# BurntSushi/aho-corasick

Hardware: NVIDIA H100
Metric: haystack_scan_throughput (higher is better)
Workload: dtype u8

## Files before the change

aho-corasick_b200/csrc/acb_api.cu:

```cuda
#include <cuda_runtime.h>

#include <algorithm>
#include <chrono>
#include <cstdio>
#include <cstdlib>
#include <cstring>
#include <atomic>
#include <pthread.h>
#include <condition_variable>
#include <functional>
#include <mutex>
#include <thread>
#include <new>
#include <vector>

#include "../../include/acb200.h"
#include "../../include/acb200_debug.h"
#include "acb_build.hpp"
#include "acb_comm.hpp"
#include "acb_device.cuh"

using acb::DfaDev;
using acb::HostDfa;

namespace {

#define CK(expr)                                                                       \
  do {                                                                                 \
    cudaError_t e_ = (expr);                                                           \
    if (e_ != cudaSuccess) {                                                           \
      std::fprintf(stderr, "acb200: CUDA error %s at %s:%d: %s\n", cudaGetErrorName(e_), \
                   __FILE__, __LINE__, cudaGetErrorString(e_));                        \
      return ACG_E_CUDA;                                                               \
    }                                                                                  \
  } while (0)

struct Workspace {
  cudaStream_t stream = nullptr, copy_stream = nullptr;
  cudaEvent_t ev0 = nullptr, ev1 = nullptr, ev2 = nullptr, ev3 = nullptr;
  uint64_t cap = 0;
  uint64_t* d_keys[2] = {nullptr, nullptr};
  uint32_t* d_pids[2] = {nullptr, nullptr};
  unsigned long long* d_counter = nullptr;
  unsigned long long* h_counter = nullptr;
  void* d_temp = nullptr;
  size_t temp_bytes = 0;
  uint64_t* h_keys = nullptr;
  uint32_t* h_pids = nullptr;
  uint64_t h_cap = 0;
  uint8_t* d_hay = nullptr;
  uint64_t d_hay_cap = 0;
  uint64_t* d_scratch = nullptr;
  uint8_t* d_flags = nullptr;
  void* d_temp2 = nullptr;
  size_t temp2_bytes = 0;
  uint64_t chain_cap = 0;
  uint64_t* d_seq = nullptr;
  uint64_t seq_cap = 0;
  uint64_t* h_seq = nullptr;
  uint64_t h_seq_cap = 0;
  acg_stats stats{};
  uint8_t* h_stage[2] = {nullptr, nullptr};
  uint64_t h_stage_cap = 0;
  cudaEvent_t stage_ev[2] = {nullptr, nullptr};
};

}

// ... 29 lines not shown
  int device = -1;
  uint32_t* d_trans = nullptr;
  uint8_t* d_classes = nullptr;
  uint32_t* d_moff = nullptr;
  uint32_t* d_mpids = nullptr;
  uint32_t* d_plens = nullptr;
  uint16_t* d_depth16 = nullptr;
  DfaDev dev{};
  int engine_override = ACG_ENGINE_AUTO;
  uint64_t pipeline_chunk = 64ull << 20;
  mutable bool bytescan_inert = false;
  uint32_t experiment = 0;
  mutable std::mutex mu;
  static constexpr size_t kMaxWorkspaces = 4;
  mutable std::vector<Workspace*> ws_all, ws_free;
  mutable std::condition_variable ws_cv;
  mutable acg_stats last_stats{};
};

namespace {

thread_local Workspace* tls_ws = nullptr;
thread_local const acg_dfa* tls_stats_owner = nullptr;
thread_local acg_stats tls_stats{};
Workspace& cur_ws() { return *tls_ws; }

int init_workspace(Workspace& w) {
  CK(cudaStreamCreateWithFlags(&w.stream, cudaStreamNonBlocking));
  CK(cudaStreamCreateWithFlags(&w.copy_stream, cudaStreamNonBlocking));
  CK(cudaEventCreate(&w.ev0));
  CK(cudaEventCreate(&w.ev1));
  CK(cudaEventCreate(&w.ev2));
  CK(cudaEventCreate(&w.ev3));
  CK(cudaMalloc(&w.d_counter, 64));
  CK(cudaMallocHost(&w.h_counter, 64));
  return ACG_OK;
}

void destroy_workspace(Workspace& w) {
  if (w.stream) cudaStreamSynchronize(w.stream);
  for (int i = 0; i < 2; ++i) { cudaFree(w.d_keys[i]); cudaFree(w.d_pids[i]); }
  cudaFree(w.d_counter); cudaFree(w.d_temp); cudaFree(w.d_hay); cudaFree(w.d_seq);
  cudaFree(w.d_scratch); cudaFree(w.d_flags); cudaFree(w.d_temp2);
  if (w.h_counter) cudaFreeHost(w.h_counter);
  if (w.h_keys) cudaFreeHost(w.h_keys);
  if (w.h_pids) cudaFreeHost(w.h_pids);
  if (w.h_seq) cudaFreeHost(w.h_seq);
  for (int i = 0; i < 2; ++i) {
    if (w.h_stage[i]) cudaFreeHost(w.h_stage[i]);
    if (w.stage_ev[i]) cudaEventDestroy(w.stage_ev[i]);
  }
  if (w.ev0) cudaEventDestroy(w.ev0);
  if (w.ev1) cudaEventDestroy(w.ev1);
  if (w.ev2) cudaEventDestroy(w.ev2);
  if (w.ev3) cudaEventDestroy(w.ev3);
  if (w.stream) cudaStreamDestroy(w.stream);
  if (w.copy_stream) cudaStreamDestroy(w.copy_stream);
}

struct WsLease {
  const acg_dfa* a;
  Workspace* w = nullptr;
  Workspace* prev;
  int rc = ACG_OK;
  explicit WsLease(const acg_dfa* a_) : a(a_), prev(tls_ws) {
    std::unique_lock<std::mutex> lk(a->mu);
    for (;;) {
      if (!a->ws_free.empty()) { w = a->ws_free.back(); a->ws_free.pop_back(); break; }
// ... 581 lines not shown
    CK(cudaEventRecord(w.ev0, w.stream));
    CK(acb::launch_walk_overlapping(a->dev, p, w.stream));
    CK(cudaEventRecord(w.ev1, w.stream));
    CK(cudaMemcpyAsync(w.h_counter, w.d_counter, 8, cudaMemcpyDeviceToHost, w.stream));
    CK(cudaStreamSynchronize(w.stream));
    cur_ws().stats.launches += 1;
    const uint64_t want = *w.h_counter;
    if (want > w.cap) { cap = want + want / 8 + 1024; continue; }
    res->n = want;
    cur_ws().stats.raw_matches = want;
    float ms = 0;
    cudaEventElapsedTime(&ms, w.ev0, w.ev1);
    cur_ws().stats.scan_ms = ms;
    if (want > 1) {
      size_t tb = w.temp_bytes;
      const int end_bit = std::min(64, acb::kTieBits + bits_for(n_bytes + 1));
      CK(cudaEventRecord(w.ev2, w.stream));
      CK(acb::sort_pairs(w.d_temp, tb, w.d_keys[0], w.d_keys[1], w.d_pids[0], w.d_pids[1], want, end_bit,
                         w.stream));
      CK(cudaEventRecord(w.ev3, w.stream));
      CK(cudaStreamSynchronize(w.stream));
      cudaEventElapsedTime(&ms, w.ev2, w.ev3);
      cur_ws().stats.order_ms = ms;
      cur_ws().stats.launches += 8;
      res->sorted_buf = 1;
    } else {
      res->sorted_buf = 0;
    }
    return ACG_OK;
  }
  return ACG_E_NOMEM;
}

int enqueue_prefilter_range(const acg_dfa* a, const uint8_t* d_hay, uint64_t readable,
                            uint64_t span_start, uint64_t span_end, uint64_t scan_lo,
                            uint64_t scan_hi, int mode, int dev_sms) {
  Workspace& w = cur_ws();
  const PrefilterPlan& pf = a->pf;
  const uintptr_t base = reinterpret_cast<uintptr_t>(d_hay);
  uint64_t lo = scan_lo + ((16 - ((base + scan_lo) & 15)) & 15);
  const uint64_t limit = std::min<uint64_t>(scan_hi, readable >= 20 ? readable - 20 : 0);
  uint64_t hi = lo;
  if (limit > lo) hi = lo + ((limit - lo) & ~15ull);
  if (lo > scan_hi) { lo = scan_hi; hi = scan_hi; }
  acb::PrefilterLaunch p;
  p.hay = d_hay;
  p.hay_len = readable;
  p.span_start = span_start;
  p.span_end = span_end;
  p.bitmap = a->d_bitmap;
  p.log_bits = pf.log_bits;
  p.k = pf.k;
  p.stride = pf.stride;
  p.geom = pf.wide ? 1 : 0;
  p.pair = 0;
  p.dyn = (a->experiment & ACG_EXP_STATIC_TILES) ? 0 : ((a->experiment & ACG_EXP_GLOBAL_TILES) ? 2 : 1);
  p.kmask = pf.kmask;
  p.fold = pf.fold;
  p.mult = pf.mult;
  p.mult3 = pf.mult3;
  p.key_shift = pf.key_shift;
  p.shift = pf.shift;
  p.dense = pf.dense ? 1 : 0;
  p.brute = pf.brute ? 1 : 0;
  p.mode = mode == 1 ? 1 : 0;
  p.first_only = mode == 2 ? 1 : 0;
  p.dup_shift = pf.dup_shift;
  p.scan_lo = scan_lo;
  p.scan_hi = scan_hi;
  p.region_lo = lo;
  p.region_hi = hi;
  p.keys = w.d_keys[0];
  p.pids = w.d_pids[0];
  p.counter = w.d_counter;
  p.cap = w.cap;
  p.bs_n = 0;
  for (int i = 0; i < 3; ++i) { p.bs_needle[i] = 0; p.bs_back[i] = 0; }
  if (pf.bs_n && !a->bytescan_inert && !(a->experiment & ACG_EXP_NO_BYTESCAN)) {
    p.bs_n = pf.bs_n;
    for (uint32_t i = 0; i < pf.bs_n; ++i) { p.bs_needle[i] = uint32_t(pf.bs_byte[i]) * 0x01010101u; p.bs_back[i] = pf.bs_back[i]; }
    CK(acb::launch_bytescan(a->dev, p, dev_sms, w.stream));
  } else {
    if (p.dyn == 2) CK(cudaMemsetAsync(w.d_counter + 2, 0, 8, w.stream));
    CK(acb::launch_prefilter(a->dev, p, dev_sms, w.stream));
  }
  cur_ws().stats.launches += 1;
  return ACG_OK;
}

int order_tuples(const acg_dfa* a, uint64_t want, uint64_t n_bytes, TupleResult* res) {
  Workspace& w = cur_ws();
  res->n = want;
  cur_ws().stats.raw_matches = want;
  if (want > 1) {
    size_t tb = w.temp_bytes;
    const int end_bit = std::min(64, acb::kTieBits + bits_for(n_bytes + 1));
    float ms = 0;
    CK(cudaEventRecord(w.ev2, w.stream));
    CK(acb::sort_pairs(w.d_temp, tb, w.d_keys[0], w.d_keys[1], w.d_pids[0], w.d_pids[1], want, end_bit,
                       w.stream));
    CK(cudaEventRecord(w.ev3, w.stream));
    CK(cudaStreamSynchronize(w.stream));
    cudaEventElapsedTime(&ms, w.ev2, w.ev3);
    cur_ws().stats.order_ms = ms;
    cur_ws().stats.launches += 8;
    res->sorted_buf = 1;
  } else {
    res->sorted_buf = 0;
  }
  return ACG_OK;
}

class CopyPool {
 public:
  static CopyPool& get() {
    static std::once_flag once;
    std::call_once(once, [] { pthread_atfork(nullptr, nullptr, [] { instance().store(nullptr); }); });
    CopyPool* p = instance().load(std::memory_order_acquire);
    if (!p) {
      CopyPool* fresh = new CopyPool;
      if (instance().compare_exchange_strong(p, fresh)) p = fresh;
    }
    return *p;
  }
  void copy(uint8_t* dst, const uint8_t* src, size_t n) {
    if (n < (4u << 20) || workers_.empty()) { std::memcpy(dst, src, n); return; }
    std::unique_lock<std::mutex> lk(mu_);
    busy_cv_.wait(lk, [&] { return !active_; });
    active_ = true;
    dst_ = dst; src_ = src; n_ = n;
    next_.store(0);
    pending_ = int(workers_.size());
    ++epoch_;
    cv_.notify_all();
    done_cv_.wait(lk, [&] { return pending_ == 0; });
    active_ = false;
    busy_cv_.notify_one();
  }

 private:
  static std::atomic<CopyPool*>& instance() {
    static std::atomic<CopyPool*> p{nullptr};
// ... 34 lines not shown
  std::atomic<size_t> next_{0};
  int pending_ = 0;
  uint64_t epoch_ = 0;
  bool active_ = false;
};

bool is_pageable_host(const void* p) {
  cudaPointerAttributes attr;
  if (cudaPointerGetAttributes(&attr, p) != cudaSuccess) { cudaGetLastError(); return false; }
  return attr.type == cudaMemoryTypeUnregistered;
}

int ensure_stage(Workspace& w, uint64_t bytes) {
  if (bytes <= w.h_stage_cap) return ACG_OK;
  for (int i = 0; i < 2; ++i) {
    if (w.h_stage[i]) { cudaFreeHost(w.h_stage[i]); w.h_stage[i] = nullptr; }
    CK(cudaMallocHost(&w.h_stage[i], bytes));
    if (!w.stage_ev[i]) CK(cudaEventCreateWithFlags(&w.stage_ev[i], cudaEventDisableTiming));
  }
  w.h_stage_cap = bytes;
  return ACG_OK;
}

int run_prefilter(const acg_dfa* a, const uint8_t* d_hay, uint64_t readable, uint64_t span_start,
                  uint64_t span_end, int mode, TupleResult* res, const uint8_t* h_hay = nullptr,
                  uint64_t scan_lo = UINT64_MAX, uint64_t scan_hi = UINT64_MAX) {
  if (scan_lo == UINT64_MAX) { scan_lo = span_start; scan_hi = span_end; }
  Workspace& w = cur_ws();
  const uint64_t n_bytes = span_end - span_start;
  if (n_bytes >= (1ull << (64 - acb::kTieBits))) return ACG_E_INVALID_ARG;
  int dev_sms = 132;
  cudaDeviceGetAttribute(&dev_sms, cudaDevAttrMultiProcessorCount, a->device);
  uint64_t cap = std::max<uint64_t>(w.cap, std::max<uint64_t>(1 << 20, (scan_hi - scan_lo) / 256));
  bool copied = h_hay == nullptr;
  for (int attempt = 0; attempt < 8; ++attempt) {
    int rc = ensure_tuple_cap(w, cap);
    if (rc) return rc;
    CK(cudaMemsetAsync(w.d_counter, 0, 16, w.stream));
    CK(cudaEventRecord(w.ev0, w.stream));
    if (copied) {
      if ((rc = enqueue_prefilter_range(a, d_hay, readable, span_start, span_end, scan_lo, scan_hi, mode,
                                        dev_sms)))
        return rc;
    } else {
      const uint64_t chunk = a->pipeline_chunk;
      const uint64_t tail = std::min<uint64_t>(a->h.max_pattern_len, 1u << 30) + 64;
      uint64_t scanned = span_start;
      const bool staged = span_end - span_start >= std::min<uint64_t>(8u << 20, chunk) && is_pageable_host(h_hay + span_start);
      if (staged && (rc = ensure_stage(w, std::min<uint64_t>(chunk, span_end - span_start)))) return rc;
      bool stage_used[2] = {false, false};
      int stage_i = 0;
      CK(cudaEventRecord(w.ev2, w.copy_stream));
      for (uint64_t c0 = span_start; c0 < span_end; c0 += chunk) {
        const uint64_t c1 = std::min(span_end, c0 + chunk);
        const uint8_t* src = h_hay + c0;
        if (staged) {
          if (stage_used[stage_i]) CK(cudaEventSynchronize(w.stage_ev[stage_i]));
          CopyPool::get().copy(w.h_stage[stage_i], h_hay + c0, size_t(c1 - c0));
          src = w.h_stage[stage_i];
        }
        CK(cudaMemcpyAsync(const_cast<uint8_t*>(d_hay) + c0, src, c1 - c0, cudaMemcpyHostToDevice,
                           w.copy_stream));
        if (staged) {
          CK(cudaEventRecord(w.stage_ev[stage_i], w.copy_stream));
          stage_used[stage_i] = true;
          stage_i ^= 1;
        }
        CK(cudaEventRecord(w.ev3, w.copy_stream));
        CK(cudaStreamWaitEvent(w.stream, w.ev3, 0));
        const uint64_t upto = c1 == span_end ? span_end : (c1 > scanned + tail ? c1 - tail : scanned);
        if (upto > scanned || c1 == span_end) {
          if ((rc = enqueue_prefilter_range(a, d_hay, c1 == span_end ? readable : c1, span_start, span_end,
                                            scanned, upto, mode, dev_sms)))
            return rc;
          scanned = upto;
        }
      }
      copied = true;
    }
    CK(cudaEventRecord(w.ev1, w.stream));
    CK(cudaMemcpyAsync(w.h_counter, w.d_counter, 16, cudaMemcpyDeviceToHost, w.stream));
    CK(cudaStreamSynchronize(w.stream));
    const uint64_t want = w.h_counter[0];
    cur_ws().stats.candidates = w.h_counter[1];
    if (a->pf.bs_n && !a->bytescan_inert && scan_hi - scan_lo >= (1u << 16) && w.h_counter[1] > (scan_hi - scan_lo) / 64)
      a->bytescan_inert = true;
    float ms = 0;
    cudaEventElapsedTime(&ms, w.ev0, w.ev1);
    cur_ws().stats.scan_ms = ms;
    if (want > w.cap) { cap = want + want / 8 + 1024; continue; }
    return order_tuples(a, want, n_bytes, res);
  }
  return ACG_E_NOMEM;
}

int ensure_chain(Workspace& w, uint64_t n) {
  if (n <= w.chain_cap) return ACG_OK;
  if (w.d_scratch) cudaFree(w.d_scratch);
  if (w.d_flags) cudaFree(w.d_flags);
  if (w.d_temp2) cudaFree(w.d_temp2);
  w.d_scratch = nullptr; w.d_flags = nullptr; w.d_temp2 = nullptr; w.chain_cap = 0;
  const uint64_t cap = std::max<uint64_t>(n, 1 << 16);
  CK(cudaMalloc(&w.d_scratch, cap * 8));
  CK(cudaMalloc(&w.d_flags, cap));
  size_t t1 = 0, t2 = 0;
  CK(acb::scan_max_u64(nullptr, t1, w.d_scratch, cap, w.stream));
  CK(acb::select_flagged(nullptr, t2, w.d_keys[0], w.d_pids[0], w.d_flags, w.d_keys[1], w.d_pids[1],
                         w.d_counter, cap, w.stream));
  w.temp2_bytes = std::max(t1, t2);
  CK(cudaMalloc(&w.d_temp2, std::max<size_t>(w.temp2_bytes, 16)));
  w.chain_cap = cap;
  return ACG_OK;
}

int run_chain(const acg_dfa* a, int mode, TupleResult* r) {
  Workspace& w = cur_ws();
  if (r->n == 0) return ACG_OK;
  int rc = ensure_chain(w, r->n);
  if (rc) return rc;
  const int src = r->sorted_buf, dst = 1 - src;
  acb::ChainLaunch c;
  c.keys = w.d_keys[src];
  c.pids = w.d_pids[src];
  c.pattern_lens = a->d_plens;
// ... 1107 lines not shown
```

aho-corasick_b200/csrc/acb_device.cuh:

```cuda
#pragma once
#include <cuda_runtime.h>
#include <stdint.h>

namespace acb {

constexpr int kTieBits = 24;
constexpr uint64_t kTieMask = (1ull << kTieBits) - 1;
constexpr uint64_t kInvalidKey = ~0ull;

struct DfaDev {
  const uint32_t* trans;
  const uint8_t* classes;
  const uint32_t* match_offsets;
  const uint32_t* match_pids;
  const uint32_t* pattern_lens;
  const uint16_t* depth16;
  uint32_t stride2;
  uint32_t max_match_id;
  uint32_t start_unanchored_id;
  uint32_t start_anchored_id;
  uint32_t max_pattern_len;
  uint32_t min_pattern_len;
  const uint2* amap;
  uint32_t amap_shift;
// ... 43 lines not shown
cudaError_t launch_seq_find(const DfaDev& dfa, const SeqLaunch& p, cudaStream_t s);

struct PrefilterLaunch {
  const uint8_t* hay;
  uint64_t hay_len;
  uint64_t span_start, span_end;
  const uint32_t* bitmap;
  uint32_t log_bits;
  uint32_t k;
  uint32_t stride;
  uint16_t geom;
  uint16_t pair;
  uint32_t kmask;
  uint32_t fold;
  uint32_t mult;
  uint32_t mult3;
  uint32_t shift;
  int dense;
  int brute;
  int mode;
  int first_only;
  uint32_t dup_shift;
  uint64_t scan_lo, scan_hi;
  uint64_t region_lo, region_hi;
  uint64_t* keys;
  uint32_t* pids;
  unsigned long long* counter;
  uint64_t cap;
  uint32_t dyn;
  uint32_t bs_n;
  uint32_t bs_needle[3];
  uint32_t bs_back[3];
  uint32_t key_shift;
};
cudaError_t launch_prefilter(const DfaDev& dfa, const PrefilterLaunch& p, int sm_count, cudaStream_t s);
cudaError_t launch_bytescan(const DfaDev& dfa, const PrefilterLaunch& p, int sm_count, cudaStream_t s);

struct ChainLaunch {
  const uint64_t* keys;
  const uint32_t* pids;
  const uint32_t* pattern_lens;
  uint64_t n;
  int mode;
  uint64_t* scratch_end;
  uint8_t* flags;
};
cudaError_t launch_chain_ends(const ChainLaunch& c, cudaStream_t s);
cudaError_t launch_chain_select(const ChainLaunch& c, cudaStream_t s);
cudaError_t scan_max_u64(void* d_temp, size_t& temp_bytes, uint64_t* data, uint64_t n, cudaStream_t s);
cudaError_t select_flagged(void* d_temp, size_t& temp_bytes, const uint64_t* keys_in, const uint32_t* pids_in,
                           const uint8_t* flags, uint64_t* keys_out, uint32_t* pids_out,
                           unsigned long long* d_num_out, uint64_t n, cudaStream_t s);

struct ExpandLaunch {
  const uint64_t* keys;
  const uint32_t* pids;
  const uint32_t* pattern_lens;
  uint64_t n;
  uint64_t first;
  uint64_t span_start;
  uint64_t offset_add;
  uint64_t* out;
  int small = 0;
};
cudaError_t launch_expand(const ExpandLaunch& e, cudaStream_t s);
cudaError_t launch_lower_bound(const uint64_t* keys, uint64_t n, uint64_t bound_key,
                               unsigned long long* d_result, cudaStream_t s);

cudaError_t sort_pairs(void* d_temp, size_t& temp_bytes, const uint64_t* keys_in, uint64_t* keys_out,
                       const uint32_t* vals_in, uint32_t* vals_out, uint64_t n, int end_bit,
                       cudaStream_t s);

}
```

aho-corasick_b200/csrc/acb_prefilter.cu:

```cuda
#include "acb_device.cuh"
#ifndef ACB_PTX_HEADER
#define ACB_PTX_HEADER "acb_ptx.cuh"
#endif
#include ACB_PTX_HEADER

#include <cstdio>
#include <cstdlib>
#include <type_traits>

#include <cub/device/device_scan.cuh>
#include <cub/device/device_select.cuh>

namespace acb {
namespace {

enum : int { kGeomNarrow = 0, kGeomWide = 1 };
template <int GEOM> struct PfGeom {
  static constexpr int kThreads = GEOM == kGeomNarrow ? 1024 : 512;
  static constexpr int kWarps = kThreads / 32;
  static constexpr int kGroups = GEOM == kGeomNarrow ? 2 : 4;
  static constexpr int kTile = kGroups * 512;
  static constexpr int kStageBytes = kTile + 16;
  static constexpr int kMinCtas = GEOM == kGeomWide ? 2 : 1;
};
// ... 6 lines not shown
  x ^= x >> 16;
  x *= 0x7feb352du;
  x ^= x >> 15;
  x *= 0x846ca68bu;
  x ^= x >> 16;
  return x;
}

__device__ __forceinline__ uint32_t bloom_hash3(uint32_t x) {
  x ^= x >> 15;
  x *= 0x2c1b3c6du;
  x ^= x >> 12;
  x *= 0x297a2d39u;
  x ^= x >> 15;
  return x;
}

#ifdef ACB_EMULATE
static const uint32_t kWinShift = getenv("ACB_EMU_WINSHIFT") ? (uint32_t)atoi(getenv("ACB_EMU_WINSHIFT")) : 31u;
#else
constexpr uint32_t kWinShift = 31;
#endif

constexpr int kPfStages = 2;

template <int GEOM, int STRIDE> struct PfPass {
  static constexpr bool kPair = STRIDE == 2 && GEOM == kGeomNarrow;
  static constexpr int kStages = kPair ? 1 : kPfStages;
  static constexpr int kGroups = PfGeom<GEOM>::kGroups * (kPair ? 2 : 1);
  static constexpr int kTile = kGroups * 512;
  static_assert(kStages * (kTile + 16) <= kPfStages * PfGeom<GEOM>::kStageBytes, "a step's tiles fit the warp's ring");
};

struct Emitter {
  uint64_t* g_keys;
  uint32_t* g_pids;
  unsigned long long* g_counter;
  uint64_t cap;
  __device__ __forceinline__ void emit(uint64_t key, uint32_t pid) {
    const unsigned m = __activemask();
    const int leader = __ffs(m) - 1;
    const int lane = threadIdx.x & 31;
    unsigned long long base = 0;
    if (lane == leader) base = atomicAdd(g_counter, (unsigned long long)__popc(m));
    base = __shfl_sync(m, base, leader);
    const unsigned long long g = base + __popc(m & ((1u << lane) - 1));
    if (g < cap) { g_keys[g] = key; g_pids[g] = pid; }
  }
};

__device__ __forceinline__ uint32_t anchor_lookup(const DfaDev& d, const PrefilterLaunch& p, uint64_t s) {
  if (s + d.amap_k > p.span_end) return 0;
  const uintptr_t a = reinterpret_cast<uintptr_t>(p.hay + s);
  const uintptr_t lo_edge = reinterpret_cast<uintptr_t>(p.hay), hi_edge = lo_edge + p.hay_len;
  const uintptr_t wa = a & ~uintptr_t(3);
  uint32_t key;
  if (wa >= lo_edge && wa + ((a & 3) ? 8 : 4) <= hi_edge) {
    const uint32_t* w = reinterpret_cast<const uint32_t*>(wa);
    const uint32_t lo = __ldg(w);
    const uint32_t hi = (a & 3) ? __ldg(w + 1) : 0u;
    key = __funnelshift_r(lo, hi, (uint32_t)(a & 3) * 8) & d.amap_kmask;
  } else {
    key = 0;
    for (uint32_t i = 0; i < d.amap_k; ++i) key |= (uint32_t)__ldg(p.hay + s + i) << (8 * i);
  }
  uint32_t slot = bloom_hash3(key) >> d.amap_shift;
  for (;;) {
    const uint2 e = __ldg(d.amap + slot);
    if (e.y == 0 || e.x == key) return e.y;
    slot = (slot + 1) & d.amap_mask;
  }
}

__device__ __forceinline__ uint32_t anchor_lookup_key(const DfaDev& d, uint32_t key) {
  uint32_t slot = bloom_hash3(key) >> d.amap_shift;
  for (;;) {
    const uint2 e = __ldg(d.amap + slot);
    if (e.y == 0 || e.x == key) return e.y;
    slot = (slot + 1) & d.amap_mask;
  }
}

template <int MODE>
__device__ __forceinline__ void verify_from(const DfaDev& d, const PrefilterLaunch& p, const uint8_t* s_cls,
                                            uint64_t s, uint32_t sid, uint32_t j, Emitter& em) {
  const uint8_t* __restrict__ hay = p.hay;
  const uint32_t* __restrict__ trans = d.trans;
  uint64_t pos = s + j;
  uint32_t best_pid = 0, best_len = 0;
  bool entered = j != 0;
  for (;;) {
    if (!entered) {
      if (pos >= p.span_end) break;
      const uint32_t b = __ldg(hay + pos);
      sid = __ldg(trans + sid + s_cls[b]);
      ++j;
      ++pos;
      if (sid == 0) break;
      if (__ldg(d.depth16 + (sid >> d.stride2)) != j) break;
    }
    entered = false;
    if (sid <= d.max_match_id) {
      const uint32_t row = sid >> d.stride2;
      const uint32_t lo = __ldg(d.match_offsets + row - 2), hi = __ldg(d.match_offsets + row - 1);
      if (MODE == 0) {
        for (uint32_t i = lo; i < hi; ++i) {
          const uint32_t pid = __ldg(d.match_pids + i);
          if (__ldg(d.pattern_lens + pid) != j) break;
          if (p.first_only && i > lo) break;
          const uint64_t tie = ((uint64_t)(d.max_pattern_len - j) << p.dup_shift) | (uint64_t)(i - lo);
          em.emit(((pos - p.span_start) << kTieBits) | tie, pid);
        }
      } else {
        const uint32_t pid = __ldg(d.match_pids + lo);
        if (__ldg(d.pattern_lens + pid) == j) { best_pid = pid; best_len = j; }
      }
    }
  }
  if (MODE == 1 && best_len) em.emit(((s - p.span_start) << kTieBits) | best_len, best_pid);
}

template <int MODE>
__device__ __forceinline__ void verify_at(const DfaDev& d, const PrefilterLaunch& p, const uint8_t* s_cls,
                                          uint64_t s, Emitter& em) {
  if (d.amap != nullptr) {
    const uint32_t sid = anchor_lookup(d, p, s);
    if (sid != 0) verify_from<MODE>(d, p, s_cls, s, sid, d.amap_k, em);
  } else {
    verify_from<MODE>(d, p, s_cls, s, d.start_unanchored_id, 0, em);
  }
}

template <int GEOM> struct PfBloom {
  static constexpr uint32_t kLogBits = GEOM == kGeomWide ? 17 : 20;
  static constexpr uint32_t kShift = 35 - kLogBits;
};

template <uint32_t SHIFT>
__device__ __forceinline__ bool bloom_test(const uint32_t* s_bitmap, uint32_t h) {
  const uint32_t byte = reinterpret_cast<const uint8_t*>(s_bitmap)[h >> SHIFT];
  const uint32_t rep = byte * 0x01010101u;
  return (__funnelshift_r(rep, rep, h) & 1u) != 0;
}

template <int MODE, bool MASKED, bool DENSE, int STRIDE, int GEOM, int DYN = 0>
__global__ void __launch_bounds__(PfGeom<GEOM>::kThreads, PfGeom<GEOM>::kMinCtas)
prefilter_kernel(DfaDev d, PrefilterLaunch p) {
  static_assert(STRIDE == 1 || STRIDE == 2, "fingerprint stride");
  static_assert(GEOM == kGeomNarrow || STRIDE == 2, "the 2 KiB tile needs the stride-2 first stage (32 hit bits per lane)");
  constexpr bool ANCH = DENSE;
  constexpr int kPfThreads = PfGeom<GEOM>::kThreads;
  constexpr int kPfWarps = PfGeom<GEOM>::kWarps;
  constexpr int kRingBytes = kPfStages * PfGeom<GEOM>::kStageBytes;
  constexpr int kStages = PfPass<GEOM, STRIDE>::kStages;
  constexpr int kPfTile = PfPass<GEOM, STRIDE>::kTile;
  constexpr int kPfStageBytes = kPfTile + 16;
  constexpr int kGroups = PfPass<GEOM, STRIDE>::kGroups;
  constexpr int kPfSlots = PfCfg<DENSE>::kSlots;
  constexpr int kSlotsAlloc = kPfSlots;
  constexpr int kPfQ2 = PfCfg<ANCH>::kQ2;
  constexpr uint32_t kBloomShift = PfBloom<GEOM>::kShift;
  using Q2Entry = typename std::conditional<ANCH, uint2, uint32_t>::type;
  ACB_DYNAMIC_SMEM(smem_raw);
  unsigned char* s_ring = smem_raw;
  uint64_t* s_bars = reinterpret_cast<uint64_t*>(s_ring + kPfWarps * kRingBytes);
  uint32_t* s_tile_of = reinterpret_cast<uint32_t*>(s_bars + kPfWarps * kPfStages);
  uint32_t* s_next_tile = s_tile_of + kPfWarps * kPfStages;
  Q2Entry* s_queue2 = reinterpret_cast<Q2Entry*>(s_next_tile + 4);
  uint16_t* s_slots = reinterpret_cast<uint16_t*>(s_queue2 + kPfWarps * kPfQ2);
  uint32_t* s_bitmap = reinterpret_cast<uint32_t*>(s_slots + kPfWarps * kSlotsAlloc);
  __shared__ uint8_t s_cls[256];

  const int tid = threadIdx.x;
  const int lane = tid & 31;
  const int warp = tid >> 5;
  const uint32_t bitmap_words = p.brute ? 0u : (1u << (p.log_bits - 5));
  for (uint32_t i = tid; i < bitmap_words; i += kPfThreads) s_bitmap[i] = p.bitmap[i];
  if (tid < 256) s_cls[tid] = d.classes[tid];
  if (tid < kPfWarps * kPfStages) ptx::mbar_init(ptx::smem_addr(&s_bars[tid]), 1);
  if (tid == 0) {
    *reinterpret_cast<uint64_t*>(s_next_tile) = DYN == 2 ? (uint64_t)blockIdx.x << 32 : 0ull;
    s_next_tile[2] = 0xFFFFFFFEu;
  }
  ptx::mbar_init_fence();
  ptx::fence_proxy_async();
  __syncthreads();

  Emitter em{p.keys, p.pids, p.counter, p.cap};
  unsigned long long cand_total = 0;

  if (blockIdx.x == 0) {
    const uint64_t tail_lo = (p.region_hi > p.region_lo && !p.brute) ? p.region_hi - (STRIDE - 1) : p.region_hi;
    const uint64_t head_n = p.region_lo - p.scan_lo;
    const uint64_t tail_n = p.scan_hi > tail_lo ? p.scan_hi - tail_lo : 0;
    for (uint64_t i = tid; i < head_n + tail_n; i += kPfThreads) {
      const uint64_t s = i < head_n ? p.scan_lo + i : tail_lo + (i - head_n);
      verify_at<MODE>(d, p, s_cls, s, em);
    }
  }

  const uint64_t n_blocks16 = (p.region_hi - p.region_lo) >> 4;
  const uint64_t per_cta = (n_blocks16 + gridDim.x - 1) / gridDim.x;
  const uint64_t b0 = (uint64_t)blockIdx.x * per_cta;
  const uint64_t b1 = min(b0 + per_cta, n_blocks16);
  const uint64_t split_lo = p.region_lo + (b0 << 4);
  const uint64_t split_hi = b0 < b1 ? p.region_lo + (b1 << 4) : split_lo;

  if (p.brute) {
    for (uint64_t s = split_lo + tid; s < split_hi; s += kPfThreads) verify_at<MODE>(d, p, s_cls, s, em);
    if (tid == 0 && split_hi > split_lo) atomicAdd(p.counter + 1, (unsigned long long)(split_hi - split_lo));
    return;
  }
  constexpr bool whole = DYN == 2;
  const uint64_t chunk_lo = whole ? p.region_lo : split_lo;
  const uint64_t chunk_hi = whole ? p.region_hi : split_hi;

  const uint32_t kmask = p.kmask, fold = p.fold, mult = p.mult;
  const uint32_t fold1 = p.fold & 0x00FFFFFFu;
  const uint32_t mult8 = p.mult3 << p.key_shift;
  const uint64_t chunk_base = chunk_lo - (uint64_t)(STRIDE - 1);
  const uint32_t rel_bias = (uint32_t)(STRIDE - 1);
// ... 292 lines not shown
            if (pass) {
              const uint32_t rel = wrel + e - j;
              if constexpr (!ANCH) q2[q2len + __popc(bal & lt)] = rel;
            }
            q2len += __popc(bal);
            if (q2len > (uint32_t)(kPfQ2 - 32)) drain2();
          }
        }
      }
    }
    __syncwarp();
    if (lane == 0) {
      if constexpr (DYN) draw(stage);
      else if (t + kStages * kPfWarps < n_tiles) issue(t + kStages * kPfWarps, stage);
    }
    if constexpr (DYN && kStages == 1) __syncwarp();
  }
  if constexpr (DYN == 2) { if (lane == 0) publish(); }
  if (q2len) drain2();
  if (lane == 0 && cand_total) atomicAdd(p.counter + 1, cand_total);
}

constexpr int kBsThreads = 512;
constexpr int kBsWarps = kBsThreads / 32;
constexpr int kBsQueue = 128;

template <int MODE>
__global__ void __launch_bounds__(kBsThreads, 2) bytescan_kernel(DfaDev d, PrefilterLaunch p) {
  __shared__ uint8_t s_cls[256];
  __shared__ uint64_t s_q[kBsWarps * kBsQueue];
  const int tid = threadIdx.x, lane = tid & 31, warp = tid >> 5;
  if (tid < 256) s_cls[tid] = d.classes[tid];
  __syncthreads();
  Emitter em{p.keys, p.pids, p.counter, p.cap};
  unsigned long long cand_total = 0;
  if (blockIdx.x == 0) {
    const uint64_t head_n = p.region_lo - p.scan_lo;
    const uint64_t tail_n = p.scan_hi > p.region_hi ? p.scan_hi - p.region_hi : 0;
    for (uint64_t i = tid; i < head_n + tail_n; i += kBsThreads)
      verify_at<MODE>(d, p, s_cls, i < head_n ? p.scan_lo + i : p.region_hi + (i - head_n), em);
  }
  uint64_t* q = s_q + warp * kBsQueue;
  uint32_t qlen = 0;
  auto drain = [&]() {
    __syncwarp();
    for (uint32_t i = lane; i < qlen; i += 32) verify_at<MODE>(d, p, s_cls, q[i], em);
    cand_total += qlen;
    qlen = 0;
    __syncwarp();
  };
  const uint32_t n_needles = p.bs_n;
  const uint32_t max_back = max(p.bs_back[0], max(p.bs_back[1], p.bs_back[2]));
  const uint32_t owned_lanes = max_back ? 31u : 32u;
  const uint64_t step_bytes = (uint64_t)owned_lanes * 16;
  const uint64_t region_bytes = p.region_hi - p.region_lo;
  const uint64_t n_steps = (region_bytes + step_bytes - 1) / step_bytes;
  const uint32_t lt = (1u << lane) - 1;
  const uint64_t load_end = p.region_hi + (max_back ? 16 : 0);
  auto load = [&](uint64_t base) -> uint4 {
    return base < load_end ? ptx::ld_nc_u4(p.hay + base) : make_uint4(0, 0, 0, 0);
  };
  auto process = [&](uint64_t base, const uint4& v) {
    const bool in_range = base < load_end;
    const uint32_t w[4] = {v.x, v.y, v.z, v.w};
    uint32_t zany = 0;
#pragma unroll
    for (int j = 0; j < 3; ++j) {
// ... 93 lines not shown
  } else {
    *e = key >> kTieBits;
    *s = *e - c.pattern_lens[c.pids[i]];
  }
}

__global__ void chain_ends_kernel(ChainLaunch c) {
  const uint64_t i = (uint64_t)blockIdx.x * blockDim.x + threadIdx.x;
  if (i >= c.n) return;
  uint64_t s, e;
  tuple_span(c, i, &s, &e);
  c.scratch_end[i] = e;
}

__global__ void chain_select_kernel(ChainLaunch c) {
  const uint64_t i = (uint64_t)blockIdx.x * blockDim.x + threadIdx.x;
  if (i >= c.n) return;
  uint64_t s, e;
  tuple_span(c, i, &s, &e);
  if (i > 0 && c.scratch_end[i - 1] > s) return;
  c.flags[i] = 1;
  uint64_t cur_end = e;
  for (uint64_t j = i + 1; j < c.n; ++j) {
    uint64_t sj, ej;
    tuple_span(c, j, &sj, &ej);
    if (c.scratch_end[j - 1] <= sj) break;
    if (sj >= cur_end) { c.flags[j] = 1; cur_end = ej; } else c.flags[j] = 0;
  }
}

struct MaxOp {
  __device__ __forceinline__ uint64_t operator()(uint64_t a, uint64_t b) const { return a > b ? a : b; }
};

}

cudaError_t launch_prefilter(const DfaDev& dfa, const PrefilterLaunch& p, int sm_count, cudaStream_t s) {
  const bool dense = p.dense != 0;
  const int geom = p.stride == 2 ? p.geom : kGeomNarrow;
  if (geom < kGeomNarrow || geom > kGeomWide) return cudaErrorInvalidValue;
  const uint32_t want_log = geom == kGeomWide ? PfBloom<kGeomWide>::kLogBits : PfBloom<kGeomNarrow>::kLogBits;
  if (!p.brute && (p.log_bits != want_log || p.shift != 35 - want_log)) return cudaErrorInvalidValue;
  const size_t bitmap_bytes = p.brute ? 0 : (size_t(1) << (p.log_bits - 3));
  static const int kThreadsOf[2] = {PfGeom<0>::kThreads, PfGeom<1>::kThreads};
  static const int kStageOf[2] = {PfGeom<0>::kStageBytes, PfGeom<1>::kStageBytes};
  const int threads = kThreadsOf[geom];
  const int warps = threads / 32;
  const int stage_bytes = kStageOf[geom];
  const int tile = geom == kGeomWide ? PfPass<kGeomWide, 2>::kTile
                   : p.stride == 2 ? PfPass<kGeomNarrow, 2>::kTile : PfPass<kGeomNarrow, 1>::kTile;
  const int q2_bytes = dense ? PfCfg<true>::kQ2 * 8 : PfCfg<false>::kQ2 * 4;
  const int slot_bytes = PfCfg<false>::kSlots * 2;
  const size_t smem = size_t(warps) * (kPfStages * stage_bytes + kPfStages * 12 + q2_bytes + slot_bytes) + 16 + bitmap_bytes;
  if (smem > 227 * 1024 - 1024) return cudaErrorInvalidValue;
  const bool masked = p.fold != 0 || p.kmask != 0xFFFFFFFFu;
  using KernT = void (*)(DfaDev, PrefilterLaunch);
#define ACB_PF_ROW(M, K, D)                                                                                 \
  {prefilter_kernel<M, K, false, 1, kGeomNarrow, D>, prefilter_kernel<M, K, true, 1, kGeomNarrow, D>, \
   prefilter_kernel<M, K, false, 2, kGeomNarrow, D>, prefilter_kernel<M, K, false, 2, kGeomWide, D>}
  static const KernT table[2][2][3][4] = {
      {{ACB_PF_ROW(0, false, 0), ACB_PF_ROW(0, false, 1), ACB_PF_ROW(0, false, 2)},
       {ACB_PF_ROW(0, true, 0), ACB_PF_ROW(0, true, 1), ACB_PF_ROW(0, true, 2)}},
      {{ACB_PF_ROW(1, false, 0), ACB_PF_ROW(1, false, 1), ACB_PF_ROW(1, false, 2)},
       {ACB_PF_ROW(1, true, 0), ACB_PF_ROW(1, true, 1), ACB_PF_ROW(1, true, 2)}}};
#undef ACB_PF_ROW
  if (p.dyn > 2) return cudaErrorInvalidValue;
// ... 11 lines not shown
  if (e != cudaSuccess) return e;
  if (per_sm < 1) per_sm = 1;
  uint64_t grid = (uint64_t)sm_count * per_sm;
  const uint64_t cta_step = uint64_t(warps) * tile;
  const uint64_t warp_steps = ((p.region_hi - p.region_lo) + cta_step - 1) / cta_step;
  if (grid > warp_steps) grid = warp_steps ? warp_steps : 1;
  ACB_LAUNCH(kern, (unsigned)grid, threads, smem, s, dfa, p);
  return cudaGetLastError();
}

cudaError_t launch_bytescan(const DfaDev& dfa, const PrefilterLaunch& p, int sm_count, cudaStream_t s) {
  if (p.bs_n < 1 || p.bs_n > 3) return cudaErrorInvalidValue;
  for (uint32_t j = 0; j < 3; ++j)
    if (p.bs_back[j] > 15) return cudaErrorInvalidValue;
  uint64_t grid = (uint64_t)sm_count * 2;
  const uint64_t steps = ((p.region_hi - p.region_lo) + 16 * 31 - 1) / (16 * 31);
  const uint64_t ctas = (steps + kBsWarps - 1) / kBsWarps;
  if (grid > ctas) grid = ctas ? ctas : 1;
  if (p.mode) ACB_LAUNCH(bytescan_kernel<1>, (unsigned)grid, kBsThreads, 0, s, dfa, p);
  else ACB_LAUNCH(bytescan_kernel<0>, (unsigned)grid, kBsThreads, 0, s, dfa, p);
  return cudaGetLastError();
}

cudaError_t launch_chain_ends(const ChainLaunch& c, cudaStream_t s) {
  const unsigned blocks = (unsigned)((c.n + 255) / 256);
  ACB_LAUNCH(chain_ends_kernel, blocks, 256, 0, s, c);
  return cudaGetLastError();
}
cudaError_t launch_chain_select(const ChainLaunch& c, cudaStream_t s) {
  const unsigned blocks = (unsigned)((c.n + 255) / 256);
  ACB_LAUNCH(chain_select_kernel, blocks, 256, 0, s, c);
  return cudaGetLastError();
}
cudaError_t scan_max_u64(void* d_temp, size_t& temp_bytes, uint64_t* data, uint64_t n, cudaStream_t s) {
  return cub::DeviceScan::InclusiveScan(d_temp, temp_bytes, data, data, MaxOp(), (int64_t)n, s);
}
cudaError_t select_flagged(void* d_temp, size_t& temp_bytes, const uint64_t* keys_in, const uint32_t* pids_in,
                           const uint8_t* flags, uint64_t* keys_out, uint32_t* pids_out,
                           unsigned long long* d_num_out, uint64_t n, cudaStream_t s) {
  size_t a = 0, b = 0;
  if (d_temp == nullptr) {
    cudaError_t e = cub::DeviceSelect::Flagged(nullptr, a, keys_in, flags, keys_out, d_num_out, (int64_t)n, s);
    if (e != cudaSuccess) return e;
    e = cub::DeviceSelect::Flagged(nullptr, b, pids_in, flags, pids_out, d_num_out, (int64_t)n, s);
    temp_bytes = a > b ? a : b;
    return e;
  }
  cudaError_t e = cub::DeviceSelect::Flagged(d_temp, temp_bytes, keys_in, flags, keys_out, d_num_out, (int64_t)n, s);
  if (e != cudaSuccess) return e;
  return cub::DeviceSelect::Flagged(d_temp, temp_bytes, pids_in, flags, pids_out, d_num_out, (int64_t)n, s);
}

}
```

Before: 1965.

## Bucket match tuples by haystack position and sort each bucket in shared memory

The prefilter emitter now places match tuples into fixed-size per-bucket regions keyed by position range. The ordering step then sorts each bucket with a block-local 8-bit radix sort in shared memory, replacing the global cub radix sort. When a bucket overflows, the code compacts the buckets and falls back to the global sort. This is meant to avoid the multi-pass global sort, at the cost of extra per-bucket counters, warp divergence in the emitter, and larger tuple buffers.

```diff
diff --git a/aho-corasick_b200/csrc/acb_api.cu b/aho-corasick_b200/csrc/acb_api.cu
--- a/aho-corasick_b200/csrc/acb_api.cu
+++ b/aho-corasick_b200/csrc/acb_api.cu
@@ -34,6 +34,8 @@
       return ACG_E_CUDA;                                                               \
     }                                                                                  \
   } while (0)
+
+constexpr size_t kCounterBytes = 8 * (acb::kBucketCountersAt + acb::kMaxBuckets);
 
 struct Workspace {
   cudaStream_t stream = nullptr, copy_stream = nullptr;
@@ -129,8 +131,8 @@
   CK(cudaEventCreate(&w.ev1));
   CK(cudaEventCreate(&w.ev2));
   CK(cudaEventCreate(&w.ev3));
-  CK(cudaMalloc(&w.d_counter, 64));
-  CK(cudaMallocHost(&w.h_counter, 64));
+  CK(cudaMalloc(&w.d_counter, kCounterBytes));
+  CK(cudaMallocHost(&w.h_counter, kCounterBytes));
   return ACG_OK;
 }
 
@@ -778,9 +780,40 @@
   return ACG_E_NOMEM;
 }
 
+struct BucketPlan {
+  uint32_t shift = 0;
+  uint32_t n = 0, log = 0, tie_bits = 0;
+  uint64_t slots() const { return uint64_t(n) << log; }
+};
+
+BucketPlan plan_buckets(const acg_dfa* a, uint64_t n_bytes) {
+  BucketPlan b;
+  if (a->experiment & ACG_EXP_GLOBAL_TILES) return b;
+  const uint32_t tie_bits = uint32_t(bits_for(a->h.max_pattern_len)) + a->pf.dup_shift;
+  if (tie_bits >= 32) return b;
+  const uint32_t max_shift = 32 - tie_bits;
+  uint32_t shift = std::min<uint32_t>(25, max_shift);
+  uint32_t min_shift = 22;
+  uint32_t log = acb::kOrderLog;
+#ifdef ACB_EMULATE
+  if (const char* e = getenv("ACB_EMU_BUCKETSHIFT")) { shift = std::min<uint32_t>(uint32_t(atoi(e)), max_shift); min_shift = 1; }
+  if (const char* e = getenv("ACB_EMU_BUCKETLOG")) log = std::min<uint32_t>(uint32_t(std::max(atoi(e), 0)), acb::kOrderLog);
+#endif
+  if (shift < min_shift) return b;
+  while ((n_bytes >> shift) + 1 > acb::kMaxBuckets) {
+    if (shift >= max_shift) return b;
+    ++shift;
+  }
+  b.shift = shift;
+  b.n = uint32_t((n_bytes >> shift) + 1);
+  b.log = log;
+  b.tie_bits = tie_bits;
+  return b;
+}
+
 int enqueue_prefilter_range(const acg_dfa* a, const uint8_t* d_hay, uint64_t readable,
                             uint64_t span_start, uint64_t span_end, uint64_t scan_lo,
-                            uint64_t scan_hi, int mode, int dev_sms) {
+                            uint64_t scan_hi, int mode, int dev_sms, const BucketPlan& bp) {
   Workspace& w = cur_ws();
   const PrefilterPlan& pf = a->pf;
   const uintptr_t base = reinterpret_cast<uintptr_t>(d_hay);
@@ -820,6 +853,9 @@
   p.pids = w.d_pids[0];
   p.counter = w.d_counter;
   p.cap = w.cap;
+  p.bucket_shift = bp.shift;
+  p.bucket_log = bp.log;
+  p.bucket_slots = bp.slots();
   p.bs_n = 0;
   for (int i = 0; i < 3; ++i) { p.bs_needle[i] = 0; p.bs_back[i] = 0; }
   if (pf.bs_n && !a->bytescan_inert && !(a->experiment & ACG_EXP_NO_BYTESCAN)) {
@@ -834,26 +870,51 @@
   return ACG_OK;
 }
 
-int order_tuples(const acg_dfa* a, uint64_t want, uint64_t n_bytes, TupleResult* res) {
+int order_tuples(const acg_dfa* a, uint64_t want, uint64_t n_bytes, TupleResult* res, const BucketPlan& bp,
+                 uint64_t overflow) {
   Workspace& w = cur_ws();
   res->n = want;
   cur_ws().stats.raw_matches = want;
-  if (want > 1) {
-    size_t tb = w.temp_bytes;
-    const int end_bit = std::min(64, acb::kTieBits + bits_for(n_bytes + 1));
-    float ms = 0;
-    CK(cudaEventRecord(w.ev2, w.stream));
+  res->sorted_buf = 0;
+  if (want <= 1 && (bp.shift == 0 || want == 0)) return ACG_OK;
+  size_t tb = w.temp_bytes;
+  const int end_bit = std::min(64, acb::kTieBits + bits_for(n_bytes + 1));
+  float ms = 0;
+  CK(cudaEventRecord(w.ev2, w.stream));
+  if (bp.shift == 0) {
     CK(acb::sort_pairs(w.d_temp, tb, w.d_keys[0], w.d_keys[1], w.d_pids[0], w.d_pids[1], want, end_bit,
                        w.stream));
-    CK(cudaEventRecord(w.ev3, w.stream));
-    CK(cudaStreamSynchronize(w.stream));
-    cudaEventElapsedTime(&ms, w.ev2, w.ev3);
-    cur_ws().stats.order_ms = ms;
     cur_ws().stats.launches += 8;
     res->sorted_buf = 1;
   } else {
-    res->sorted_buf = 0;
-  }
+    acb::OrderLaunch o;
+    o.keys_in = w.d_keys[0];
+    o.pids_in = w.d_pids[0];
+    o.keys_out = w.d_keys[1];
+    o.pids_out = w.d_pids[1];
+    o.bucket_count = w.d_counter + acb::kBucketCountersAt;
+    o.overflow_count = w.d_counter;
+    o.n_buckets = bp.n;
+    o.bucket_shift = bp.shift;
+    o.bucket_cap = 1u << bp.log;
+    o.tie_bits = bp.tie_bits;
+    o.bucket_slots = bp.slots();
+    if (overflow == 0) {
+      CK(acb::launch_order_buckets(o, w.stream));
+      cur_ws().stats.launches += 1;
+      res->sorted_buf = 1;
+    } else {
+      CK(acb::launch_compact_buckets(o, w.stream));
+      CK(acb::sort_pairs(w.d_temp, tb, w.d_keys[1], w.d_keys[0], w.d_pids[1], w.d_pids[0], want, end_bit,
+                         w.stream));
+      cur_ws().stats.launches += 9;
+      res->sorted_buf = 0;
+    }
+  }
+  CK(cudaEventRecord(w.ev3, w.stream));
+  CK(cudaStreamSynchronize(w.stream));
+  cudaEventElapsedTime(&ms, w.ev2, w.ev3);
+  cur_ws().stats.order_ms = ms;
   return ACG_OK;
 }
 
@@ -954,15 +1015,18 @@
   int dev_sms = 132;
   cudaDeviceGetAttribute(&dev_sms, cudaDevAttrMultiProcessorCount, a->device);
   uint64_t cap = std::max<uint64_t>(w.cap, std::max<uint64_t>(1 << 20, (scan_hi - scan_lo) / 256));
+  const BucketPlan bp = plan_buckets(a, n_bytes);
+  cap = std::max<uint64_t>(cap, bp.slots() + (bp.shift ? (1u << 16) : 0));
+  const size_t counter_bytes = bp.shift ? 8 * (acb::kBucketCountersAt + size_t(bp.n)) : 16;
   bool copied = h_hay == nullptr;
   for (int attempt = 0; attempt < 8; ++attempt) {
     int rc = ensure_tuple_cap(w, cap);
     if (rc) return rc;
-    CK(cudaMemsetAsync(w.d_counter, 0, 16, w.stream));
+    CK(cudaMemsetAsync(w.d_counter, 0, counter_bytes, w.stream));
     CK(cudaEventRecord(w.ev0, w.stream));
     if (copied) {
       if ((rc = enqueue_prefilter_range(a, d_hay, readable, span_start, span_end, scan_lo, scan_hi, mode,
-                                        dev_sms)))
+                                        dev_sms, bp)))
         return rc;
     } else {
       const uint64_t chunk = a->pipeline_chunk;
@@ -993,7 +1057,7 @@
         const uint64_t upto = c1 == span_end ? span_end : (c1 > scanned + tail ? c1 - tail : scanned);
         if (upto > scanned || c1 == span_end) {
           if ((rc = enqueue_prefilter_range(a, d_hay, c1 == span_end ? readable : c1, span_start, span_end,
-                                            scanned, upto, mode, dev_sms)))
+                                            scanned, upto, mode, dev_sms, bp)))
             return rc;
           scanned = upto;
         }
@@ -1001,17 +1065,27 @@
       copied = true;
     }
     CK(cudaEventRecord(w.ev1, w.stream));
-    CK(cudaMemcpyAsync(w.h_counter, w.d_counter, 16, cudaMemcpyDeviceToHost, w.stream));
+    CK(cudaMemcpyAsync(w.h_counter, w.d_counter, counter_bytes, cudaMemcpyDeviceToHost, w.stream));
     CK(cudaStreamSynchronize(w.stream));
-    const uint64_t want = w.h_counter[0];
+    uint64_t want = w.h_counter[0], overflow = 0, room = w.cap;
+    if (bp.shift) {
+      overflow = want;
+      want = 0;
+      for (uint32_t i = 0; i < bp.n; ++i) want += w.h_counter[acb::kBucketCountersAt + i];
+      room = w.cap - bp.slots();
+    }
     cur_ws().stats.candidates = w.h_counter[1];
     if (a->pf.bs_n && !a->bytescan_inert && scan_hi - scan_lo >= (1u << 16) && w.h_counter[1] > (scan_hi - scan_lo) / 64)
       a->bytescan_inert = true;
     float ms = 0;
     cudaEventElapsedTime(&ms, w.ev0, w.ev1);
     cur_ws().stats.scan_ms = ms;
-    if (want > w.cap) { cap = want + want / 8 + 1024; continue; }
-    return order_tuples(a, want, n_bytes, res);
+    if (bp.shift ? overflow > room : want > w.cap) {
+      const uint64_t need = bp.shift ? overflow : want;
+      cap = (w.cap - room) + need + need / 8 + 1024;
+      continue;
+    }
+    return order_tuples(a, want, n_bytes, res, bp, overflow);
   }
   return ACG_E_NOMEM;
 }
diff --git a/aho-corasick_b200/csrc/acb_device.cuh b/aho-corasick_b200/csrc/acb_device.cuh
--- a/aho-corasick_b200/csrc/acb_device.cuh
+++ b/aho-corasick_b200/csrc/acb_device.cuh
@@ -99,6 +99,9 @@
   uint32_t bs_needle[3];
   uint32_t bs_back[3];
   uint32_t key_shift;
+  uint32_t bucket_shift;
+  uint32_t bucket_log;
+  uint64_t bucket_slots;
 };
 cudaError_t launch_prefilter(const DfaDev& dfa, const PrefilterLaunch& p, int sm_count, cudaStream_t s);
 cudaError_t launch_bytescan(const DfaDev& dfa, const PrefilterLaunch& p, int sm_count, cudaStream_t s);
@@ -134,6 +137,24 @@
 cudaError_t launch_lower_bound(const uint64_t* keys, uint64_t n, uint64_t bound_key,
                                unsigned long long* d_result, cudaStream_t s);
 
+constexpr int kBucketCountersAt = 8;
+constexpr uint32_t kMaxBuckets = 1024;
+constexpr uint32_t kOrderLog = 14;
+constexpr uint32_t kOrderCap = 1u << kOrderLog;
+struct OrderLaunch {
+  const uint64_t* keys_in;
+  const uint32_t* pids_in;
+  uint64_t* keys_out;
+  uint32_t* pids_out;
+  const unsigned long long* bucket_count;
+  const unsigned long long* overflow_count;
+  uint32_t n_buckets, bucket_shift, bucket_cap;
+  uint32_t tie_bits;
+  uint64_t bucket_slots;
+};
+cudaError_t launch_order_buckets(const OrderLaunch& o, cudaStream_t s);
+cudaError_t launch_compact_buckets(const OrderLaunch& o, cudaStream_t s);
+
 cudaError_t sort_pairs(void* d_temp, size_t& temp_bytes, const uint64_t* keys_in, uint64_t* keys_out,
                        const uint32_t* vals_in, uint32_t* vals_out, uint64_t n, int end_bit,
                        cudaStream_t s);
diff --git a/aho-corasick_b200/csrc/acb_prefilter.cu b/aho-corasick_b200/csrc/acb_prefilter.cu
--- a/aho-corasick_b200/csrc/acb_prefilter.cu
+++ b/aho-corasick_b200/csrc/acb_prefilter.cu
@@ -62,20 +62,40 @@
   static_assert(kStages * (kTile + 16) <= kPfStages * PfGeom<GEOM>::kStageBytes, "a step's tiles fit the warp's ring");
 };
 
+template <bool BUCKETED = true>
 struct Emitter {
   uint64_t* g_keys;
   uint32_t* g_pids;
   unsigned long long* g_counter;
   uint64_t cap;
+  uint32_t bucket_shift, bucket_log;
+  uint64_t bucket_slots;
   __device__ __forceinline__ void emit(uint64_t key, uint32_t pid) {
     const unsigned m = __activemask();
     const int leader = __ffs(m) - 1;
     const int lane = threadIdx.x & 31;
-    unsigned long long base = 0;
-    if (lane == leader) base = atomicAdd(g_counter, (unsigned long long)__popc(m));
-    base = __shfl_sync(m, base, leader);
-    const unsigned long long g = base + __popc(m & ((1u << lane) - 1));
-    if (g < cap) { g_keys[g] = key; g_pids[g] = pid; }
+    const bool bucketed = BUCKETED && bucket_shift != 0;
+    unsigned long long* cnt = g_counter;
+    uint64_t first = 0;
+    bool together = true;
+    if (bucketed) {
+      const uint32_t b = (uint32_t)(key >> (kTieBits + bucket_shift));
+      cnt += kBucketCountersAt + b;
+      first = (uint64_t)b << bucket_log;
+      together = __ballot_sync(m, b == (uint32_t)__shfl_sync(m, b, leader)) == m;
+    }
+    unsigned long long g;
+    if (together) {
+      unsigned long long base = 0;
+      if (lane == leader) base = atomicAdd(cnt, (unsigned long long)__popc(m));
+      base = __shfl_sync(m, base, leader);
+      g = base + __popc(m & ((1u << lane) - 1));
+    } else {
+      g = atomicAdd(cnt, 1ull);
+    }
+    uint64_t slot = first + g;
+    if (bucketed && g >> bucket_log) slot = bucket_slots + atomicAdd(g_counter, 1ull);
+    if (slot < cap) { g_keys[slot] = key; g_pids[slot] = pid; }
   }
 };
 
@@ -111,9 +131,9 @@
   }
 }
 
-template <int MODE>
+template <int MODE, class EM>
 __device__ __forceinline__ void verify_from(const DfaDev& d, const PrefilterLaunch& p, const uint8_t* s_cls,
-                                            uint64_t s, uint32_t sid, uint32_t j, Emitter& em) {
+                                            uint64_t s, uint32_t sid, uint32_t j, EM& em) {
   const uint8_t* __restrict__ hay = p.hay;
   const uint32_t* __restrict__ trans = d.trans;
   uint64_t pos = s + j;
@@ -150,9 +170,9 @@
   if (MODE == 1 && best_len) em.emit(((s - p.span_start) << kTieBits) | best_len, best_pid);
 }
 
-template <int MODE>
+template <int MODE, class EM>
 __device__ __forceinline__ void verify_at(const DfaDev& d, const PrefilterLaunch& p, const uint8_t* s_cls,
-                                          uint64_t s, Emitter& em) {
+                                          uint64_t s, EM& em) {
   if (d.amap != nullptr) {
     const uint32_t sid = anchor_lookup(d, p, s);
     if (sid != 0) verify_from<MODE>(d, p, s_cls, s, sid, d.amap_k, em);
@@ -216,7 +236,7 @@
   ptx::fence_proxy_async();
   __syncthreads();
 
-  Emitter em{p.keys, p.pids, p.counter, p.cap};
+  Emitter<DYN != 2> em{p.keys, p.pids, p.counter, p.cap, p.bucket_shift, p.bucket_log, p.bucket_slots};
   unsigned long long cand_total = 0;
 
   if (blockIdx.x == 0) {
@@ -575,7 +595,7 @@
   const int tid = threadIdx.x, lane = tid & 31, warp = tid >> 5;
   if (tid < 256) s_cls[tid] = d.classes[tid];
   __syncthreads();
-  Emitter em{p.keys, p.pids, p.counter, p.cap};
+  Emitter<> em{p.keys, p.pids, p.counter, p.cap, p.bucket_shift, p.bucket_log, p.bucket_slots};
   unsigned long long cand_total = 0;
   if (blockIdx.x == 0) {
     const uint64_t head_n = p.region_lo - p.scan_lo;
@@ -735,6 +755,157 @@
 struct MaxOp {
   __device__ __forceinline__ uint64_t operator()(uint64_t a, uint64_t b) const { return a > b ? a : b; }
 };
+
+constexpr int kOrdThreads = 1024;
+constexpr int kOrdWarps = kOrdThreads / 32;
+constexpr int kOrdRounds = (int)kOrderCap / kOrdThreads;
+constexpr int kOrdBatch = 8;
+
+__global__ void __launch_bounds__(kOrdThreads, 1) order_buckets_kernel(OrderLaunch o) {
+  ACB_DYNAMIC_SMEM(smem_raw);
+  const uint32_t cap = o.bucket_cap;
+  uint32_t* ka = reinterpret_cast<uint32_t*>(smem_raw);
+  uint32_t* kb = ka + cap;
+  uint16_t* ia = reinterpret_cast<uint16_t*>(kb + cap);
+  uint16_t* ib = ia + cap;
+  uint16_t* s_cnt = ib + cap;
+  uint32_t* s_sum = reinterpret_cast<uint32_t*>(s_cnt + 256 * kOrdWarps);
+  const int tid = threadIdx.x, lane = tid & 31, warp = tid >> 5;
+  const uint32_t lt = (1u << lane) - 1;
+  const uint32_t b = blockIdx.x;
+  const uint32_t n = (uint32_t)o.bucket_count[b];
+  if (n == 0) return;
+
+  uint32_t part = 0;
+  for (uint32_t i = tid; i < b; i += kOrdThreads) part += (uint32_t)o.bucket_count[i];
+  part = __reduce_add_sync(0xffffffffu, part);
+  if (lane == 0) s_sum[warp] = part;
+  __syncthreads();
+  uint64_t out0 = 0;
+  for (int w = 0; w < kOrdWarps; ++w) out0 += s_sum[w];
+
+  const uint64_t in0 = (uint64_t)b * cap;
+  const uint64_t off0 = (uint64_t)b << o.bucket_shift;
+  const uint32_t tie_bits = o.tie_bits;
+  const uint64_t tie_mask = (1ull << tie_bits) - 1;
+  for (uint32_t j0 = 0; j0 < n; j0 += kOrdBatch * kOrdThreads) {
+    uint64_t k[kOrdBatch];
+#pragma unroll
+    for (int u = 0; u < kOrdBatch; ++u) {
+      const uint32_t j = j0 + u * kOrdThreads + tid;
+      k[u] = j < n ? o.keys_in[in0 + j] : 0;
+    }
+#pragma unroll
+    for (int u = 0; u < kOrdBatch; ++u) {
+      const uint32_t j = j0 + u * kOrdThreads + tid;
+      if (j < n) {
+        ka[j] = (uint32_t)((((k[u] >> kTieBits) - off0) << tie_bits) | (k[u] & tie_mask));
+        ia[j] = (uint16_t)j;
+      }
+    }
+  }
+
+  const uint32_t per_warp = (n + kOrdWarps - 1) / kOrdWarps;
+  const uint32_t w_lo = min(warp * per_warp, n), w_hi = min(w_lo + per_warp, n);
+  const uint32_t rounds = (per_warp + 31) / 32;
+  const uint32_t key_bits = o.bucket_shift + tie_bits;
+  for (uint32_t sh = 0; sh < key_bits; sh += 8) {
+    for (int i = tid; i < 256 * kOrdWarps / 2; i += kOrdThreads) reinterpret_cast<uint32_t*>(s_cnt)[i] = 0;
+    __syncthreads();
+    uint32_t rd[kOrdRounds];
+#pragma unroll
+    for (int r = 0; r < kOrdRounds; ++r) {
+      rd[r] = 0;
+      if ((uint32_t)r < rounds) {
+        const uint32_t i = w_lo + r * 32 + lane;
+        const bool valid = i < w_hi;
+        const uint32_t digit = valid ? (ka[i] >> sh) & 0xFFu : 0u;
+        uint32_t peers = __ballot_sync(0xffffffffu, valid);
+#pragma unroll
+        for (int bit = 0; bit < 8; ++bit) {
+          const uint32_t bb = __ballot_sync(0xffffffffu, (digit >> bit) & 1u);
+          peers &= ((digit >> bit) & 1u) ? bb : ~bb;
+        }
+        uint16_t* c = s_cnt + digit * kOrdWarps + warp;
+        const uint32_t base = valid ? *c : 0u;
+        __syncwarp();
+        if (valid && (peers & lt) == 0) *c = (uint16_t)(base + __popc(peers));
+        __syncwarp();
+        rd[r] = (digit << 16) | (base + __popc(peers & lt));
+      }
+    }
+    __syncthreads();
+    {
+      constexpr int kPer = 256 * kOrdWarps / kOrdThreads;
+      uint16_t* c = s_cnt + tid * kPer;
+      uint32_t v[kPer], sum = 0;
+#pragma unroll
+      for (int u = 0; u < kPer; ++u) { v[u] = c[u]; sum += v[u]; }
+      uint32_t incl = sum;
+#pragma unroll
+      for (int d = 1; d < 32; d <<= 1) {
+        const uint32_t x = (uint32_t)__shfl_sync(0xffffffffu, incl, lane >= d ? lane - d : lane);
+        if (lane >= d) incl += x;
+      }
+      if (lane == 31) s_sum[warp] = incl;
+      __syncthreads();
+      uint32_t run = incl - sum;
+      for (int w = 0; w < warp; ++w) run += s_sum[w];
+#pragma unroll
+      for (int u = 0; u < kPer; ++u) { c[u] = (uint16_t)run; run += v[u]; }
+    }
+    __syncthreads();
+#pragma unroll
+    for (int r = 0; r < kOrdRounds; ++r) {
+      const uint32_t i = w_lo + r * 32 + lane;
+      if ((uint32_t)r < rounds && i < w_hi) {
+        const uint32_t dst = s_cnt[(rd[r] >> 16) * kOrdWarps + warp] + (rd[r] & 0xFFFFu);
+        kb[dst] = ka[i];
+        ib[dst] = ia[i];
+      }
+    }
+    __syncthreads();
+    uint32_t* tk = ka; ka = kb; kb = tk;
+    uint16_t* ti = ia; ia = ib; ib = ti;
+  }
+
+  for (uint32_t j0 = 0; j0 < n; j0 += kOrdBatch * kOrdThreads) {
+    uint32_t pid[kOrdBatch];
+#pragma unroll
+    for (int u = 0; u < kOrdBatch; ++u) {
+      const uint32_t j = j0 + u * kOrdThreads + tid;
+      pid[u] = j < n ? o.pids_in[in0 + ia[j]] : 0u;
+    }
+#pragma unroll
+    for (int u = 0; u < kOrdBatch; ++u) {
+      const uint32_t j = j0 + u * kOrdThreads + tid;
+      if (j < n) {
+        const uint32_t sk = ka[j];
+        o.keys_out[out0 + j] = ((off0 + (sk >> tie_bits)) << kTieBits) | (sk & tie_mask);
+        o.pids_out[out0 + j] = pid[u];
+      }
+    }
+  }
+}
+
+constexpr int kCompactThreads = 256;
+__global__ void __launch_bounds__(kCompactThreads) compact_buckets_kernel(OrderLaunch o) {
+  __shared__ unsigned long long s_part[kCompactThreads];
+  const uint32_t b = blockIdx.x;
+  const int tid = threadIdx.x;
+  unsigned long long part = 0;
+  for (uint32_t i = tid; i < b && i < o.n_buckets; i += kCompactThreads) part += min(o.bucket_count[i], (unsigned long long)o.bucket_cap);
+  s_part[tid] = part;
+  __syncthreads();
+  uint64_t dst = 0;
+  for (int i = 0; i < kCompactThreads; ++i) dst += s_part[i];
+  const uint64_t n = b < o.n_buckets ? min(o.bucket_count[b], (unsigned long long)o.bucket_cap) : *o.overflow_count;
+  const uint64_t src = b < o.n_buckets ? (uint64_t)b * o.bucket_cap : o.bucket_slots;
+  for (uint64_t j = tid; j < n; j += kCompactThreads) {
+    o.keys_out[dst + j] = o.keys_in[src + j];
+    o.pids_out[dst + j] = o.pids_in[src + j];
+  }
+}
 
 }
 
@@ -812,7 +983,21 @@
   ACB_LAUNCH(chain_select_kernel, blocks, 256, 0, s, c);
   return cudaGetLastError();
 }
-cudaError_t scan_max_u64(void* d_temp, size_t& temp_bytes, uint64_t* data, uint64_t n, cudaStream_t s) {
+cudaError_t launch_order_buckets(const OrderLaunch& o, cudaStream_t s) {
+  if (o.n_buckets == 0 || o.n_buckets > kMaxBuckets || o.bucket_cap == 0 || o.bucket_cap > kOrderCap ||
+      o.bucket_shift + o.tie_bits > 32)
+    return cudaErrorInvalidValue;
+  const size_t smem = size_t(o.bucket_cap) * 12 + 256 * kOrdWarps * 2 + kOrdWarps * 4;
+  cudaError_t e = cudaFuncSetAttribute(order_buckets_kernel, cudaFuncAttributeMaxDynamicSharedMemorySize, (int)smem);
+  if (e != cudaSuccess) return e;
+  ACB_LAUNCH(order_buckets_kernel, o.n_buckets, kOrdThreads, smem, s, o);
+  return cudaGetLastError();
+}
+cudaError_t launch_compact_buckets(const OrderLaunch& o, cudaStream_t s) {
+  ACB_LAUNCH(compact_buckets_kernel, o.n_buckets + 1, kCompactThreads, 0, s, o);
+  return cudaGetLastError();
+}
+cudaError_t scan_max_u64(void* d_temp,size_t& temp_bytes, uint64_t* data, uint64_t n, cudaStream_t s) {
   return cub::DeviceScan::InclusiveScan(d_temp, temp_bytes, data, data, MaxOp(), (int64_t)n, s);
 }
 cudaError_t select_flagged(void* d_temp, size_t& temp_bytes, const uint64_t* keys_in, const uint32_t* pids_in,
```

Result: faster. 2102, median of 6 (+7.0%).
